# AzheeeQAQ/Game-of-life-distributed

Hardware: AMD Instinct MI355X
Metric: cell-updates/sec (GCUPS) at 1/2/4/8 MI355X; % of HBM roofline (higher is better)
Workload: dtype u32 bit-sliced (1 bit/cell)

## Files before the change

game-of-life-distributed_amd/csrc/gol_kernels.hip:

```cpp
#include "gol_kernels.h"
#include "gol_bits.h"
#include "gol_layout.h"

#include <algorithm>
#include <climits>
#include <type_traits>
#include <utility>

namespace golk {
#ifndef GOL_LOOP_PAD
#define GOL_LOOP_PAD 0
#endif
#ifndef GOL_FILL_PHASES
#define GOL_FILL_PHASES 4
#endif

template <typename F, int... I>
__device__ __forceinline__ void static_for_impl(F &&f, std::integer_sequence<int, I...>) {
    (f(std::integral_constant<int, I>()), ...);
}
template <int N, typename F>
__device__ __forceinline__ void static_for(F &&f) {
    static_for_impl(f, std::make_integer_sequence<int, N>());
}
// ... 447 lines not shown
        if ((threadIdx.x & 63) == 0) atomicAdd(a.alive, (unsigned long long)tot);
    }
}

template <int D, int WPL, bool CNT>
__global__ __launch_bounds__(512) void gol_tb_pair_kernel(StepArgs a) {
    const int lane = threadIdx.x & 63;
    const int w = __builtin_amdgcn_readfirstlane(threadIdx.x >> 6);
    const int tiles_x = (a.Ww + tile_words(WPL) - 1) / tile_words(WPL);
    const int S = a.rows_per_wave;
    const int q = blockIdx.x * 4 + (w & 3);
    const int region = q / tiles_x;
    const int tile = q - region * tiles_x;
    const int r0 = region * 2 * S;
    const int len = r0 < a.rows_out ? min(2 * S, a.rows_out - r0) : 0;
    __shared__ int s_claim[4];
    __shared__ unsigned long long s_cnt;
    if (w < 4 && lane == 0) s_claim[w] = len;
    if (CNT && threadIdx.x == 0) s_cnt = 0;
    __syncthreads();
    if (len == 0) return;
    const uint32_t cnt = stream_band<D, true, WPL, pair_store<WPL>(), true, pair_g2<WPL>()>(a, r0, len, tile * tile_words(WPL), blockIdx.x * 8 + w,
                                                   w < 4 ? 1 : -1, &s_claim[w & 3]);
    if constexpr (!CNT) {
        if (a.alive) {
            const uint32_t tot = wave_sum_u32(cnt);
            if (lane == 0 && tot) atomicAdd(a.alive, (unsigned long long)tot);
        }
    } else if (a.alive) {
        const uint32_t tot = wave_sum_u32(cnt);
        int active = 0;
        for (int i = 0; i < 4; ++i) {
            const int qi = blockIdx.x * 4 + i;
            active += (qi / tiles_x) * 2 * S < a.rows_out ? 2 : 0;
        }
        if (lane == 0) {
            const unsigned long long mine = (1ull << 40) | tot;
            const unsigned long long now = atomicAdd(&s_cnt, mine) + mine;
            const unsigned long long sum = now & ((1ull << 40) - 1);
            if ((int)(now >> 40) == active && sum) atomicAdd(a.alive, sum);
        }
    }
}

__device__ __forceinline__ void wg_count(unsigned long long *alive, unsigned long long *s_cnt, uint32_t cnt, int active) {
    const uint32_t tot = wave_sum_u32(cnt);
    if ((threadIdx.x & 63) == 0) {
        const unsigned long long mine = (1ull << 40) | tot;
        const unsigned long long now = atomicAdd(s_cnt, mine) + mine;
        const unsigned long long sum = now & ((1ull << 40) - 1);
        if ((int)(now >> 40) == active && sum) atomicAdd(alive, sum);
    }
}

template <int WPL>
__device__ __forceinline__ void put_lanes(uint32_t *row, const uint32_t (&v)[WPL]) {
    const int lane = threadIdx.x & 63;
    if constexpr (WPL == 1)
        row[lane] = v[0];
    else if constexpr (WPL == 2)
        reinterpret_cast<uint2 *>(row)[lane] = make_uint2(v[0], v[1]);
    else
        reinterpret_cast<uint4 *>(row)[lane] = make_uint4(v[0], v[1], v[2], v[3]);
}
template <int WPL>
__device__ __forceinline__ Lanes<WPL> get_lanes(const uint32_t *row) {
    const int lane = threadIdx.x & 63;
    Lanes<WPL> v;
    if constexpr (WPL == 1) {
        v.w[0] = row[lane];
    } else if constexpr (WPL == 2) {
        const uint2 q = reinterpret_cast<const uint2 *>(row)[lane];
        v.w[0] = q.x;
        v.w[1] = q.y;
    } else {
        const uint4 q = reinterpret_cast<const uint4 *>(row)[lane];
        v.w[0] = q.x;
        v.w[1] = q.y;
        v.w[2] = q.z;
        v.w[3] = q.w;
    }
    return v;
}
template <int WPL>
__device__ __forceinline__ Lanes<WPL> load_row(const uint32_t *p) {
    Lanes<WPL> v;
    if constexpr (WPL == 1) {
        v.w[0] = *p;
    } else if constexpr (WPL == 2) {
        const uint2 q = *reinterpret_cast<const uint2 *>(p);
        v.w[0] = q.x;
        v.w[1] = q.y;
    } else {
        const uint4 q = *reinterpret_cast<const uint4 *>(p);
        v.w[0] = q.x;
        v.w[1] = q.y;
        v.w[2] = q.z;
        v.w[3] = q.w;
    }
    return v;
}
template <int D, int A, int WPL, typename Hook>
__device__ __forceinline__ void push_group_exp(Lanes<WPL> &x0, Lanes<WPL> &x1, Lanes<WPL> &x2,
                                               uint32_t (&h0)[3][D][WPL], uint32_t (&h1)[3][D][WPL],
                                               uint32_t (&cc)[3][D][WPL], int ii0, Hook &&hook) {
    parity_fix<1>();
#pragma unroll
    for (int s = 0; s < A + 2; ++s) {
        if constexpr (WPL <= 2) parity_fix<1>();
        if (s < A) {
            hook(s, ii0, x0);
            stage<D, 0, WPL>(s, x0, h0, h1, cc);
        }
        if (s >= 1 && s - 1 < A) {
            hook(s - 1, ii0 + 1, x1);
            stage<D, 1, WPL>(s - 1, x1, h0, h1, cc);
        }
        if (s >= 2 && s - 2 < A) {
            hook(s - 2, ii0 + 2, x2);
            stage<D, 2, WPL>(s - 2, x2, h0, h1, cc);
        }
    }
}
#ifndef GOL_SKEW_WAIT_TRACE
#define GOL_SKEW_WAIT_TRACE 0
#endif
#ifndef GOL_SKEW_STORE_CPOL
#define GOL_SKEW_STORE_CPOL 16
#endif
template <int D>
struct SkewPlan {
    static constexpr int STEP = D > 20 ? 6 : 3;
    static constexpr int NPH = (D - 1) / STEP;
    static constexpr int P(int j) { return (j + 1) * STEP; }
    static constexpr int NROWS(int j) { return 2 * ((j + 1 < NPH ? P(j + 1) : D) - P(j)); }
    static constexpr int BASE(int j) {
        int b = 0;
        for (int i = 0; i < j; ++i) b += NROWS(i);
        return b;
    }
    static constexpr int NEXP = BASE(NPH);
    static_assert(NPH >= 1 && STEP % 3 == 0, "skew depth >= 4");
};


template <int D, int WPL>
struct PairSt {
    uint32_t a0[D][WPL], a1[D][WPL];
    uint32_t b0[D][WPL], b1[D][WPL];
    uint32_t p0[D][WPL], p1[D][WPL], p2[D][WPL];
    uint32_t c[D][WPL];
};

template <int D, int PH, int WPL>
__device__ __forceinline__ void stage_pr(int t, Lanes<WPL> &x, PairSt<D, WPL> &st) {
    uint32_t west[WPL], east[WPL];
    if constexpr (WPL == 1) {
        const uint32_t l = from_left_lane(x.w[0]);
        const uint32_t r = from_right_lane(x.w[0]);
        west[0] = __builtin_amdgcn_alignbit(x.w[0], l, 31);
        east[0] = __builtin_amdgcn_alignbit(r, x.w[0], 1);
    } else if constexpr (WPL == 4) {
        const uint32_t l3 = from_left_lane(x.w[3]);
        const uint32_t r0 = from_right_lane(x.w[0]);
        west[0] = __builtin_amdgcn_alignbit(x.w[3], l3, 31);
        west[1] = x.w[0];
        west[2] = x.w[1];
        west[3] = x.w[2];
        east[0] = x.w[1];
        east[1] = x.w[2];
        east[2] = x.w[3];
        east[3] = __builtin_amdgcn_alignbit(r0, x.w[0], 1);
    } else {
        const uint32_t l1 = from_left_lane(x.w[1]);
        const uint32_t r0 = from_right_lane(x.w[0]);
        west[0] = __builtin_amdgcn_alignbit(x.w[1], l1, 31);
        east[0] = x.w[1];
        west[1] = x.w[0];
        east[1] = __builtin_amdgcn_alignbit(r0, x.w[0], 1);
    }
    uint32_t nx[WPL];
#pragma unroll
    for (int k = 0; k < WPL; ++k) {
        const uint32_t n0 = bop<kXor3>(west[k], x.w[k], east[k]);
        const uint32_t n1 = bop<kMaj>(west[k], x.w[k], east[k]);
        if constexpr (PH == 1) {
            uint32_t p0, p1, p2;
            pair_sum(st.b0[t][k], st.b1[t][k], n0, n1, p0, p1, p2);
            nx[k] = pair_rule(st.a0[t][k], st.a1[t][k], p0, p1, p2, st.c[t][k]);
            st.p0[t][k] = p0;
            st.p1[t][k] = p1;
            st.p2[t][k] = p2;
            st.a0[t][k] = n0;
            st.a1[t][k] = n1;
        } else {
            nx[k] = pair_rule(n0, n1, st.p0[t][k], st.p1[t][k], st.p2[t][k], st.c[t][k]);
            st.b0[t][k] = n0;
            st.b1[t][k] = n1;
        }
    }
#pragma unroll
    for (int k = 0; k < WPL; ++k) {
        st.c[t][k] = x.w[k];
        x.w[k] = nx[k];
    }
}

template <int D, int KQ, int WPL>
__device__ __forceinline__ void push_group_pr(Lanes<WPL> &x0, Lanes<WPL> &x1, Lanes<WPL> &x2,
                                              PairSt<D, WPL> &st) {
    parity_fix<1>();
    static_for<D + 2>([&](auto s_tag) {
        constexpr int s = decltype(s_tag)::value;
        parity_fix<2>();
        if constexpr (s < D) stage_pr<D, (KQ + 0 + s) & 1, WPL>(s, x0, st);
        if constexpr (s >= 1 && s - 1 < D) stage_pr<D, (KQ + 1 + s - 1) & 1, WPL>(s - 1, x1, st);
        if constexpr (s >= 2) stage_pr<D, (KQ + 2 + s - 2) & 1, WPL>(s - 2, x2, st);
    });
}

template <int D, int KQ, int LO, int WPL>
__device__ __forceinline__ void push_group_pr_hi(Lanes<WPL> &x0, Lanes<WPL> &x1, Lanes<WPL> &x2,
                                                 PairSt<D, WPL> &st) {
    parity_fix<1>();
    static_for<D + 2>([&](auto s_tag) {
        constexpr int s = decltype(s_tag)::value;
        if constexpr (s >= LO) {
            parity_fix<2>();
            if constexpr (s < D) stage_pr<D, (KQ + 0 + s) & 1, WPL>(s, x0, st);
            if constexpr (s - 1 >= LO && s - 1 < D) stage_pr<D, (KQ + 1 + s - 1) & 1, WPL>(s - 1, x1, st);
            if constexpr (s - 2 >= LO) stage_pr<D, (KQ + 2 + s - 2) & 1, WPL>(s - 2, x2, st);
        }
    });
}

template <int D, int KQ, int WPL>
__device__ __forceinline__ void pr_enter(const uint32_t (&h0)[3][D][WPL], const uint32_t (&h1)[3][D][WPL],
                                         const uint32_t (&cc)[3][D][WPL], PairSt<D, WPL> &st) {
#pragma unroll
    for (int t = 0; t < D; ++t)
#pragma unroll
        for (int k = 0; k < WPL; ++k) {
            st.c[t][k] = cc[2][t][k];
            if (((KQ + t) & 1) == 1) {
                st.a0[t][k] = h0[1][t][k];
                st.a1[t][k] = h1[1][t][k];
                st.b0[t][k] = h0[2][t][k];
                st.b1[t][k] = h1[2][t][k];
            } else {
                pair_sum(h0[1][t][k], h1[1][t][k], h0[2][t][k], h1[2][t][k], st.p0[t][k], st.p1[t][k], st.p2[t][k]);
                st.a0[t][k] = h0[2][t][k];
                st.a1[t][k] = h1[2][t][k];
            }
        }
}
template <int D, int KQ, int WPL>
__device__ __forceinline__ void pr_leave(const PairSt<D, WPL> &st, uint32_t (&h0)[3][D][WPL],
                                         uint32_t (&h1)[3][D][WPL], uint32_t (&cc)[3][D][WPL]) {
#pragma unroll
    for (int t = 0; t < D; ++t)
#pragma unroll
        for (int k = 0; k < WPL; ++k) {
            cc[2][t][k] = st.c[t][k];
            if (((KQ + t) & 1) == 1) {
                h0[1][t][k] = st.a0[t][k];
                h1[1][t][k] = st.a1[t][k];
                h0[2][t][k] = st.b0[t][k];
                h1[2][t][k] = st.b1[t][k];
            } else {
                h0[2][t][k] = st.a0[t][k];
                h1[2][t][k] = st.a1[t][k];
                pair_unsum(st.p0[t][k], st.p1[t][k], st.a0[t][k], st.a1[t][k], h0[1][t][k], h1[1][t][k]);
            }
        }
}

template <int D, int LO, int WPL>
__device__ __forceinline__ void push_group_hi(Lanes<WPL> &x0, Lanes<WPL> &x1, Lanes<WPL> &x2,
                                              uint32_t (&h0)[3][D][WPL], uint32_t (&h1)[3][D][WPL],
                                              uint32_t (&cc)[3][D][WPL]) {
    parity_fix<1>();
#pragma unroll
    for (int s = LO; s < D + 2; ++s) {
        parity_fix<2>();
        if (s < D) stage<D, 0, WPL>(s, x0, h0, h1, cc);
        if (s - 1 >= LO && s - 1 < D) stage<D, 1, WPL>(s - 1, x1, h0, h1, cc);
        if (s - 2 >= LO) stage<D, 2, WPL>(s - 2, x2, h0, h1, cc);
    }
}

template <int D, int WPL, bool HALF = false, bool PR = false>
__device__ __forceinline__ uint32_t stream_skew(const StepArgs &a, int ab, int eb, int tile, bool self,
                                                uint32_t *exp_mine, const uint32_t *exp_next, int *flag_mine,
                                                int *flag_next, unsigned *error, unsigned long long *phase_tr,
                                                int dr = 0) {
    using SP = SkewPlan<D>;
    constexpr int ROW = 64 * WPL;
    constexpr int TV = HALF ? kHalfTileValid : kTileValid;
    const int lane = threadIdx.x & 63;
    const int hl = HALF ? (lane & 31) : lane;
    const int rofs = (HALF && lane >= 32) ? dr : 0;
    const int Ww = a.Ww;
    const int S = eb - ab;
    const int t0 = tile * TV * WPL;
    int col = (t0 + WPL * (hl - 1)) % Ww;
    if (col < 0) col += Ww;
    const bool keep = hl >= 1 && hl <= TV && (t0 + WPL * (hl - 1)) < Ww;
    int r = ab + rofs + a.in.off;
    const int wrap = a.in.wrap > 0 ? a.in.wrap : INT_MAX;
    if (a.in.wrap > 0) {
        r %= a.in.wrap;
        if (r < 0) r += a.in.wrap;
    }
    const uint32_t *__restrict__ src = a.src + col;
    auto load_next = [&]() -> Lanes<WPL> {
        const Lanes<WPL> v = load_row<WPL>(src + (size_t)(a.in.base + min(r, a.in.rmax)) * Ww);
        r = (r + 1 == wrap) ? 0 : r + 1;
        return v;
    };
    const __amdgpu_buffer_rsrc_t brs = __builtin_amdgcn_make_buffer_rsrc(
        a.dst + (size_t)(a.dst_base + ab + D) * Ww, (short)0, (S + (HALF ? dr : 0)) * Ww * 4, 0x00020000);
    const int clo = a.count_lo - (ab + D + rofs), chi = a.count_hi - (ab + D + rofs);
    const int colw = col + rofs * Ww;
    uint32_t cnt = 0;
    auto emit = [&](const Lanes<WPL> &y, int oi) {
        const bool ok = keep && (unsigned)oi < (unsigned)S;
        const int off = ok ? (oi * Ww + colw) * 4 : INT_MAX;
        if constexpr (WPL == 1)
            __builtin_amdgcn_raw_buffer_store_b32(y.w[0], brs, off, 0, GOL_SKEW_STORE_CPOL);
        else if constexpr (WPL == 2)
            __builtin_amdgcn_raw_buffer_store_b64((__attribute__((ext_vector_type(2))) unsigned){y.w[0], y.w[1]}, brs,
                                                  off, 0, GOL_SKEW_STORE_CPOL);
        else
            __builtin_amdgcn_raw_buffer_store_b128(
                (__attribute__((ext_vector_type(4))) unsigned){y.w[0], y.w[1], y.w[2], y.w[3]}, brs, off, 0,
                GOL_SKEW_STORE_CPOL);
        uint32_t pc = 0;
#pragma unroll
        for (int k = 0; k < WPL; ++k) pc += __builtin_popcount(y.w[k]);
        cnt += (ok && oi >= clo && oi < chi) ? pc : 0u;
    };
    auto hook = [&](int s, int k, const Lanes<WPL> &x) {
        if (s % SP::STEP != 0 || s == 0 || s / SP::STEP > SP::NPH) return;
        const int j = s / SP::STEP - 1;
        const int m = k - 2 * SP::P(j);
        const int row = (unsigned)m < (unsigned)SP::NROWS(j) ? SP::BASE(j) + m : SP::NEXP;
        put_lanes<WPL>(exp_mine + row * ROW, x.w);
    };

    uint32_t h0[3][D][WPL], h1[3][D][WPL], cc[3][D][WPL];
#pragma unroll
    for (int s = 0; s < 3; ++s)
#pragma unroll
        for (int t = 0; t < D; ++t)
#pragma unroll
            for (int k = 0; k < WPL; ++k) h0[s][t][k] = h1[s][t][k] = cc[s][t][k] = 0u;

    Lanes<WPL> x0 = vmov(load_next()), x1 = vmov(load_next()), x2 = vmov(load_next());
    int k = 0;
    [[maybe_unused]] unsigned long long wt0 = 0, wmain = 0, nmain = 0, wfill = 0, nfill = 0;
    auto fill = [&](auto a_tag) {
        constexpr int A = decltype(a_tag)::value;
        for (; A == D ? k <= 2 * D - 1 : (k + 2) / 2 <= A - 1; k += 3) {
            const Lanes<WPL> n0 = load_next(), n1 = load_next(), n2 = load_next();
            __builtin_amdgcn_sched_barrier(0);
            Lanes<WPL> y0 = x0, y1 = x1, y2 = x2;
            push_group_exp<D, A, WPL>(y0, y1, y2, h0, h1, cc, k, hook);
            if constexpr (A == D) {
                emit(y0, k - 2 * D);
                emit(y1, k + 1 - 2 * D);
                emit(y2, k + 2 - 2 * D);
            }
            __builtin_amdgcn_sched_barrier(0);
            if constexpr (GOL_SKEW_WAIT_TRACE) wt0 = __builtin_amdgcn_s_memrealtime();
            x0 = vmov(n0);
            x1 = vmov(n1);
            x2 = vmov(n2);
            if constexpr (GOL_SKEW_WAIT_TRACE) {
                asm volatile("s_waitcnt vmcnt(0)" ::: "memory");
                wfill += __builtin_amdgcn_s_memrealtime() - wt0;
                ++nfill;
            }
        }
    };
    static_for<SP::NPH>([&](auto j) { fill(std::integral_constant<int, SP::P(decltype(j)::value)>()); });
    fill(std::integral_constant<int, D>());
    if (phase_tr && lane == 0) phase_tr[0] = (unsigned long long)__builtin_amdgcn_s_memrealtime();
    asm volatile("s_waitcnt lgkmcnt(0)" ::: "memory");
    if (lane == 0) __hip_atomic_store(flag_mine, 1, __ATOMIC_RELAXED, __HIP_MEMORY_SCOPE_WORKGROUP);

    Lanes<WPL> q0, q1, q2;
#pragma unroll
    for (int i = 0; i < WPL; ++i) q0.w[i] = q1.w[i] = q2.w[i] = 0u;
    int qoi = -8;
    [[maybe_unused]] PairSt<D, WPL> st;
    const int kmain = S + (self ? 2 * D : 2 * SP::P(0));
    for (int i = 0; i < GOL_LOOP_PAD; ++i) asm volatile("s_nop 0");
    if constexpr (PR) {
        constexpr int KSTART = 3 * ((2 * D + 2) / 3);
        static_assert(KSTART % 6 == 0, "the pair main loop starts at an even push");
        {
            pr_enter<D, 0, WPL>(h0, h1, cc, st);
            for (; k < kmain; k += 6) {
                {
                    const Lanes<WPL> n0 = load_next(), n1 = load_next(), n2 = load_next();
                    emit(q0, qoi);
                    emit(q1, qoi + 1);
                    emit(q2, qoi + 2);
                    __builtin_amdgcn_sched_barrier(0);
                    Lanes<WPL> y0 = x0, y1 = x1, y2 = x2;
                    push_group_pr<D, 0, WPL>(y0, y1, y2, st);
                    q0 = y0;
                    q1 = y1;
                    q2 = y2;
                    qoi = k - 2 * D;
                    __builtin_amdgcn_sched_barrier(0);
                    x0 = vmov(n0);
                    x1 = vmov(n1);
                    x2 = vmov(n2);
                }
                {
                    const Lanes<WPL> n0 = load_next(), n1 = load_next(), n2 = load_next();
                    emit(q0, qoi);
                    emit(q1, qoi + 1);
                    emit(q2, qoi + 2);
                    __builtin_amdgcn_sched_barrier(0);
                    Lanes<WPL> y0 = x0, y1 = x1, y2 = x2;
                    push_group_pr<D, 1, WPL>(y0, y1, y2, st);
                    q0 = y0;
                    q1 = y1;
                    q2 = y2;
                    qoi = k + 3 - 2 * D;
                    __builtin_amdgcn_sched_barrier(0);
                    x0 = vmov(n0);
                    x1 = vmov(n1);
                    x2 = vmov(n2);
                }
            }
            if constexpr (D % 3 != 0) pr_leave<D, 0, WPL>(st, h0, h1, cc);
        }
    }
    for (; !PR && k < kmain; k += 3) {
        const Lanes<WPL> n0 = load_next(), n1 = load_next(), n2 = load_next();
        emit(q0, qoi);
        emit(q1, qoi + 1);
        emit(q2, qoi + 2);
        __builtin_amdgcn_sched_barrier(0);
        Lanes<WPL> y0 = x0, y1 = x1, y2 = x2;
        push_group<D, D, WPL>(y0, y1, y2, h0, h1, cc);
        q0 = y0;
        q1 = y1;
        q2 = y2;
        qoi = k - 2 * D;
        __builtin_amdgcn_sched_barrier(0);
        if constexpr (GOL_SKEW_WAIT_TRACE) wt0 = __builtin_amdgcn_s_memrealtime();
        x0 = vmov(n0);
        x1 = vmov(n1);
        x2 = vmov(n2);
        if constexpr (GOL_SKEW_WAIT_TRACE) {
            asm volatile("s_waitcnt vmcnt(3)" ::: "memory");
            wmain += __builtin_amdgcn_s_memrealtime() - wt0;
            ++nmain;
        }
    }
    if constexpr (GOL_SKEW_WAIT_TRACE) {
        if (phase_tr && lane == 0) {
            phase_tr[32] = wmain;
            phase_tr[33] = nmain;
            phase_tr[64] = wfill;
            phase_tr[65] = nfill;
        }
    }
    if (phase_tr && lane == 0) phase_tr[1] = (unsigned long long)__builtin_amdgcn_s_memrealtime();
    if (!self) {
        if (__hip_atomic_load(flag_next, __ATOMIC_RELAXED, __HIP_MEMORY_SCOPE_WORKGROUP) == 0) {
            const long long t_start = (long long)__builtin_amdgcn_s_memrealtime();
            while (__hip_atomic_load(flag_next, __ATOMIC_RELAXED, __HIP_MEMORY_SCOPE_WORKGROUP) == 0) {
                if ((long long)__builtin_amdgcn_s_memrealtime() - t_start > 200000000ll) {
                    if (error && lane == 0) __hip_atomic_store(error, 1u, __ATOMIC_RELAXED, __HIP_MEMORY_SCOPE_SYSTEM);
                    break;
                }
                __builtin_amdgcn_s_sleep(1);
            }
        }
        asm volatile("s_waitcnt lgkmcnt(0)" ::: "memory");
        auto imports = [&](int kg, Lanes<WPL> &y0, Lanes<WPL> &y1, Lanes<WPL> &y2) {
            const int d = kg - S;
            int base = SP::BASE(0) - 2 * SP::P(0);
            static_for<SP::NPH>([&](auto j) {
                constexpr int J = decltype(j)::value;
                if (J > 0 && d >= 2 * SP::P(J)) base = SP::BASE(J) - 2 * SP::P(J);
            });
            const int top = SP::NEXP - 1;
            y0 = get_lanes<WPL>(exp_next + min(base + d, top) * ROW);
            y1 = get_lanes<WPL>(exp_next + min(base + d + 1, top) * ROW);
            y2 = get_lanes<WPL>(exp_next + min(base + d + 2, top) * ROW);
        };
        {
            Lanes<WPL> n0, n1, n2;
            imports(k, n0, n1, n2);
            x0 = vmov(n0);
            x1 = vmov(n1);
            x2 = vmov(n2);
        }
        auto drain_pr = [&](auto kq_tag, auto lo_tag) {
            constexpr int KQ = decltype(kq_tag)::value, LO = decltype(lo_tag)::value;
            Lanes<WPL> n0, n1, n2;
            imports(k + 3, n0, n1, n2);
            __builtin_amdgcn_sched_barrier(0);
            Lanes<WPL> y0 = x0, y1 = x1, y2 = x2;
            push_group_pr_hi<D, KQ, LO, WPL>(y0, y1, y2, st);
            parity_fix<1>();
            emit(q0, qoi);
            emit(q1, qoi + 1);
            emit(q2, qoi + 2);
            q0 = y0;
            q1 = y1;
            q2 = y2;
            qoi = k - 2 * D;
            __builtin_amdgcn_sched_barrier(0);
            x0 = vmov(n0);
            x1 = vmov(n1);
            x2 = vmov(n2);
            k += 3;
        };
        auto drain = [&](auto lo_tag, int kend) {
            constexpr int LO = decltype(lo_tag)::value;
            if constexpr (PR && D % 3 == 0) {
                if constexpr (LO == SP::P(SP::NPH - 1) && D - LO <= 6) {
                    static_for<(D - LO) / 3>([&](auto) {
                        drain_pr(std::integral_constant<int, 0>(), lo_tag);
                        drain_pr(std::integral_constant<int, 1>(), lo_tag);
                    });
                    return;
                }
                while (k < kend) {
                    drain_pr(std::integral_constant<int, 0>(), lo_tag);
                    drain_pr(std::integral_constant<int, 1>(), lo_tag);
                }
                return;
            }
            for (; k < kend; k += 3) {
                Lanes<WPL> n0, n1, n2;
                imports(k + 3, n0, n1, n2);
                __builtin_amdgcn_sched_barrier(0);
                Lanes<WPL> y0 = x0, y1 = x1, y2 = x2;
                push_group_hi<D, LO, WPL>(y0, y1, y2, h0, h1, cc);
                __builtin_amdgcn_sched_barrier(0);
                emit(q0, qoi);
                emit(q1, qoi + 1);
                emit(q2, qoi + 2);
                q0 = y0;
                q1 = y1;
                q2 = y2;
                qoi = k - 2 * D;
                __builtin_amdgcn_sched_barrier(0);
                x0 = vmov(n0);
                x1 = vmov(n1);
                x2 = vmov(n2);
            }
        };
        static_for<SP::NPH>([&](auto j) {
            constexpr int J = decltype(j)::value;
            drain(std::integral_constant<int, SP::P(J)>(), S + 2 * (J + 1 < SP::NPH ? SP::P(J + 1) : D));
        });
    }
    emit(q0, qoi);
    emit(q1, qoi + 1);
    emit(q2, qoi + 2);
    return cnt;
}

template <int D, int WPL, bool HALF = false, bool PR = false>
__global__ __launch_bounds__(512) void gol_skew_kernel(SkewArgs p) {
    using SP = SkewPlan<D>;
    constexpr int ROW = 64 * WPL;
    __shared__ uint32_t s_exp[8][(SP::NEXP + 1) * ROW];
    __shared__ int s_flag[8];
    __shared__ unsigned long long s_cnt;
    const int lane = threadIdx.x & 63;
    const int w = __builtin_amdgcn_readfirstlane(threadIdx.x >> 6);
    const int sy = 8 / p.tx;
    const int tcols = (p.tiles_x + p.tx - 1) / p.tx;
    const int stack = blockIdx.x / tcols, tc = blockIdx.x - stack * tcols;
    const int tile = tc * p.tx + w % p.tx, pos = w / p.tx;
    if (lane == 0) s_flag[w] = 0;
    if (threadIdx.x == 0) s_cnt = 0;
    __syncthreads();
    if (tile >= p.tiles_x) return;
    if (p.prio_young && w >= 4) __builtin_amdgcn_s_setprio(1);
    const int L = HALF ? p.base.rows_out / 2 : p.base.rows_out;
    const int A0 = (int)((int64_t)stack * L / p.nst) - D, E0 = (int)((int64_t)(stack + 1) * L / p.nst) - D;
    const int64_t Ls = (int64_t)(E0 - A0) + p.hcap;
    int cum = 0, tot = 0;
    for (int q = 0; q < sy; ++q) {
        tot += p.wgt[q];
        cum += q < pos ? p.wgt[q] : 0;
    }
    const bool bottom = pos == sy - 1;
    constexpr int G = PR ? 6 : 3;
    const int ab = A0 + (int)(Ls * cum / tot) / G * G;
    const int eb = bottom ? E0 : A0 + (int)(Ls * (cum + p.wgt[pos]) / tot) / G * G;
    const long long t_start = p.trace ? (long long)__builtin_amdgcn_s_memrealtime() : 0;
    const uint32_t cnt = stream_skew<D, WPL, HALF, PR>(p.base, ab, eb, tile, bottom, s_exp[w], bottom ? nullptr : s_exp[w + p.tx],
                                             &s_flag[w], bottom ? nullptr : &s_flag[w + p.tx], p.error,
                                             (p.trace && blockIdx.x < 1024) ? p.trace + 8 + 2 * (blockIdx.x * 64 + 16 + w)
                                                                            : nullptr,
                                             L);
    if (p.trace && lane == 0 && blockIdx.x < 1024) {
        p.trace[8 + 2 * (blockIdx.x * 64 + w)] = (unsigned long long)t_start;
        p.trace[8 + 2 * (blockIdx.x * 64 + w) + 1] = (unsigned long long)__builtin_amdgcn_s_memrealtime();
    }
    if (p.base.alive) wg_count(p.base.alive, &s_cnt, cnt, sy * min(p.tx, p.tiles_x - tc * p.tx));
}

__host__ __device__ constexpr int persist_waves(int depth, int wpl) { return depth * wpl <= 16 ? 16 : 8; }

#ifndef GOL_PERSIST_WG_COUNT
#define GOL_PERSIST_WG_COUNT 1
#endif
template <int D, int WPL, int NW>
__global__ __launch_bounds__(NW * 64) void gol_persist_kernel(PersistArgs p) {
    const int lane = threadIdx.x & 63;
    const int w = __builtin_amdgcn_readfirstlane(threadIdx.x >> 6);
    const int b = blockIdx.x;
    const int wx = b % p.cols, wy = b / p.cols;
    const int tile = wx * p.wg_tx + w % p.wg_tx;
    int r0, band, dir = 1;
    const int ry = w / p.wg_tx;
    const bool paired = p.paired != 0;
    if (paired) {
        const int hr = p.wg_sy / 2;
        r0 = wy * p.wg_sy * p.S + 2 * (ry % hr) * p.S;
        band = 2 * p.S;
        dir = ry < hr ? 1 : -1;
    } else if (p.S_old > 0) {
        const int hr = p.wg_sy / 2;
        const int base = wy * p.wg_sy * p.S;
        r0 = base + (ry < hr ? ry * p.S_old : hr * p.S_old + (ry - hr) * p.S_young);
        band = ry < hr ? p.S_old : p.S_young;
        if (ry == p.wg_sy - 1) band = base + p.wg_sy * p.S - r0;
    } else {
        r0 = (wy * p.wg_sy + ry) * p.S;
        band = p.S;
    }
    const int rows_here = (tile < p.tiles_x && r0 < p.base.rows_out) ? min(band, p.base.rows_out - r0) : 0;

    int nb = b;
    if (lane < 9) {
        const int ny = (wy + lane / 3 - 1 + p.wg_y) % p.wg_y;
        const int nx = (wx + lane % 3 - 1 + p.cols) % p.cols;
        nb = ny * p.cols + nx;
    }
    __shared__ int s_abort;
    __shared__ int s_claim[2][NW / 2];
#if GOL_PERSIST_WG_COUNT
    __shared__ unsigned long long s_cnt;
    if (threadIdx.x == 0) s_cnt = 0;
#endif
    if (threadIdx.x == 0) s_abort = 0;
    if (paired && w < NW / 2 && lane == 0) s_claim[0][w] = rows_here;
    __syncthreads();

    uint32_t cnt = 0;
    long long tr_wait = 0, tr_band = 0, tr_max = 0;
    const long long tr_t0 = (long long)__builtin_amdgcn_s_memrealtime();
    for (int j = 0; j < p.J; ++j) {
        const long long tr_w0 = (long long)__builtin_amdgcn_s_memrealtime();
        if (j > 0) {
            if (w == NW - 1) {
                const long long t_start = (long long)__builtin_amdgcn_s_memrealtime();
                for (;;) {
                    const unsigned v = __hip_atomic_load(&p.progress[nb], __ATOMIC_RELAXED, __HIP_MEMORY_SCOPE_AGENT);
                    if (__all(v >= (unsigned)j)) break;
// ... 1635 lines not shown
```

game-of-life-distributed_amd/csrc/golhip.hip:

```cpp
#include <hip/hip_runtime.h>
#include <rccl/rccl.h>

#include <algorithm>
#include <climits>
#include <functional>
#include <atomic>
#include <cstdarg>
#include <cstdio>
#include <cstring>
#include <mutex>
#include <string>
#include <vector>

#include "../../include/golhip.h"
#include "gol_kernels.h"

using golk::kHalo;

namespace {

thread_local std::string g_err;

struct HostBuf {
    uintptr_t base;
// ... 454 lines not shown
    h->ev_pending.clear();
    return GOLHIP_OK;
}

void plan(int strip_rows, int nranks, int rank, int depth, int Ww, golhip_halo_plan_t *p) {
    p->prev_rank = (rank - 1 + nranks) % nranks;
    p->next_rank = (rank + 1) % nranks;
    p->rows = depth;
    p->send_up_row = kHalo;
    p->recv_bottom_row = kHalo + strip_rows;
    p->send_down_row = kHalo + strip_rows - depth;
    p->recv_top_row = kHalo - depth;
    p->bytes = (int64_t)depth * Ww * 4;
}

int exchange_rccl(golhip_t h, int depth, hipStream_t st) {
    if (h->halo_skip) return GOLHIP_OK;
    golhip_halo_plan_t p;
    plan(h->rows, h->nranks, h->rank, depth, h->Ww, &p);
    uint32_t *b = h->buf[h->cur];
    const size_t n = (size_t)depth * h->Ww;
    hipEvent_t e0 = nullptr, e1 = nullptr;
    if (h->flags & GOLHIP_FLAG_TIMING) {
        e0 = take_event(h);
        e1 = take_event(h);
        if (!e0 || !e1) return fail(GOLHIP_EHIP, "hipEventCreate failed");
        HIP_OR_FAIL(hipEventRecord(e0, st));
    }
    if (h->xport) {
        if ((int64_t)n > h->xport_cap) {
            HIP_OR_FAIL(hipHostFree(h->xport_host));
            h->xport_host = nullptr;
            h->xport_cap = 0;
            HIP_OR_FAIL(hipHostMalloc(&h->xport_host, 4 * n * 4, hipHostMallocDefault));
            h->xport_cap = (int64_t)n;
        }
        uint32_t *hb = h->xport_host;
        const size_t bytes = n * 4;
        HIP_OR_FAIL(hipMemcpyAsync(hb, b + (int64_t)p.send_up_row * h->Ww, bytes, hipMemcpyDeviceToHost, st));
        HIP_OR_FAIL(hipMemcpyAsync(hb + n, b + (int64_t)p.send_down_row * h->Ww, bytes, hipMemcpyDeviceToHost, st));
        HIP_OR_FAIL(hipStreamSynchronize(st));
        if (int r = h->xport(h->xport_user, p.prev_rank, p.next_rank, hb, hb + n, hb + 2 * n, hb + 3 * n,
                             (int64_t)bytes))
            return fail(GOLHIP_ERCCL, "test transport returned %d", r);
        HIP_OR_FAIL(hipMemcpyAsync(b + (int64_t)p.recv_top_row * h->Ww, hb + 2 * n, bytes, hipMemcpyHostToDevice, st));
        HIP_OR_FAIL(hipMemcpyAsync(b + (int64_t)p.recv_bottom_row * h->Ww, hb + 3 * n, bytes, hipMemcpyHostToDevice, st));
        HIP_OR_FAIL(hipStreamSynchronize(st));
    } else {
        NCCL_OR_FAIL(ncclGroupStart());
        NCCL_OR_FAIL(ncclSend(b + (int64_t)p.send_up_row * h->Ww, n, ncclUint32, p.prev_rank, h->comm, st));
        NCCL_OR_FAIL(ncclRecv(b + (int64_t)p.recv_bottom_row * h->Ww, n, ncclUint32, p.next_rank, h->comm, st));
        NCCL_OR_FAIL(ncclSend(b + (int64_t)p.send_down_row * h->Ww, n, ncclUint32, p.next_rank, h->comm, st));
        NCCL_OR_FAIL(ncclRecv(b + (int64_t)p.recv_top_row * h->Ww, n, ncclUint32, p.prev_rank, h->comm, st));
        NCCL_OR_FAIL(ncclGroupEnd());
    }
    if (e1) {
        HIP_OR_FAIL(hipEventRecord(e1, st));
        h->ev_pending.push_back({e0, e1, 3});
    }
    h->halo_bytes += 2 * (int64_t)n * 4;
    h->halo_exchanges++;
    return GOLHIP_OK;
}

void shift_rows(golk::StepArgs &a, int lo, int hi) {
    const int rows = a.rows_out;
    a.rows_out = hi - lo;
    a.dst_base = kHalo + lo;
    a.in.off = kHalo + lo;
    a.dummy_rows = std::max(1, std::min(a.dummy_rows, kHalo + std::min(lo, 0)));
    a.count_lo = -lo;
    a.count_hi = -lo + rows;
}

int skew_bpc(golhip_t h, int depth, int wpl, bool half, bool pr) {
    int &c = h->skew_bpc[depth_index(depth)][(wpl == 4 ? 2 : wpl - 1) + (half ? 3 : 0) + (pr ? 6 : 0)];
    if (c == 0) {
        const int b = golk::skew_blocks_per_cu(depth, wpl, half, pr);
        c = b > 0 ? b : -1;
    }
    return c;
}

bool skew_dims(golhip_t h, int depth, int wpl, int L, golk::SkewArgs *sk) {
    const bool pr = depth == 18 || (wpl == 4 && depth == 8 && (h->skew_pairs & 2));
    if (!h->skew || h->W % 32 != 0 || !golk::skew_supported(depth, wpl, false, pr)) return false;
    const int hcap = h->skew_hcap >= 0 ? h->skew_hcap : 3 * depth / 4;
    const int smin = depth + 3;
    const bool half_ok = h->skew_half >= 0 && L % 2 == 0 && golk::skew_supported(depth, wpl, true, pr);
    int best_tx = 0, best_nst = 0, best_half = 0, best_tiles = 0;
    double best = 1e300;
    for (int half = 0; half <= (half_ok ? 1 : 0); ++half) {
        if (!half && half_ok && h->skew_half > 0) continue;
        const int bpc = skew_bpc(h, depth, wpl, half, pr);
        if (bpc < 1) continue;
        const int tiles = half ? (h->Ww + golk::kHalfTileValid * wpl - 1) / (golk::kHalfTileValid * wpl)
                               : golk::tb_tiles(h->Ww, wpl);
        const int Lh = half ? L / 2 : L;
        for (int tx = 1; tx <= 2; ++tx) {
            if (h->skew_tx && tx != h->skew_tx) continue;
            const int sy = 8 / tx, tcols = (tiles + tx - 1) / tx;
            const int nst = std::min(h->cu_count * bpc / tcols,
                                     Lh / (sy * (smin + hcap) - hcap));
            if (nst < 1) continue;
            if (h->skew == 1 && (int64_t)nst * tcols * 4 < (int64_t)h->cu_count * bpc * 3) continue;
            if (((double)Lh / nst + hcap + (half ? Lh : 0)) * h->Ww * 4 >= 2147483648.0) continue;
            const double per_wave = ((double)Lh / nst + hcap) / sy * (half ? 1.02 : 1.0);
            if (per_wave < best * 0.999) {
                best = per_wave;
                best_tx = tx;
                best_nst = nst;
                best_half = half;
                best_tiles = tiles;
            }
        }
    }
    if (!best_tx) return false;
    sk->tiles_x = best_tiles;
    sk->pairs = pr ? 1 : 0;
    sk->tx = best_tx;
    sk->nst = best_nst;
    sk->half = best_half;
    sk->hcap = hcap;
    return true;
}

bool skew_fills(golhip_t h) {
    if (!h->skew || h->W % 32 != 0) return false;
    const int wpl = wpl_per_launch(h);
    int cap = std::min(h->tb_depth, golk::max_depth_for(wpl));
    if (cap == 9 && wpl != 4) cap = 8;
    const int depth = cap == 9 ? 9 : largest_depth(cap);
    golk::SkewArgs sk{};
    return skew_dims(h, depth, wpl, sched_rows(h), &sk);
}

bool skew_plan(golhip_t h, int depth, int wpl, const golk::StepArgs &a, golk::SkewArgs *sk) {
    if (!skew_dims(h, depth, wpl, a.rows_out, sk)) return false;
    if (!h->skew_err) {
        void *p = nullptr, *d = nullptr;
        if (hipHostMalloc(&p, sizeof(unsigned), hipHostMallocMapped) != hipSuccess) return false;
        if (hipHostGetDevicePointer(&d, p, 0) != hipSuccess) {
            (void)hipHostFree(p);
            return false;
        }
        h->skew_err = static_cast<unsigned *>(p);
        h->skew_err_dev = static_cast<unsigned *>(d);
        *h->skew_err = 0;
    }
    const int sy = 8 / sk->tx;
    const int young = h->skew_young > 0 ? h->skew_young
                      : wpl == 4             ? 78
                      : sk->half             ? 60
                      : a.in.wrap > 0        ? 70
                                             : 68;
    for (int q = 0; q < 8; ++q) sk->wgt[q] = (q < sy && q * sk->tx >= 4) ? young : 100;
    sk->prio_young = h->skew_prio;
    sk->error = h->skew_err_dev;
    sk->trace = h->d_trace;
    return true;
}

int launch_rows(golhip_t h, int depth, unsigned long long *alive, bool halo, int lo, int hi) {
    const hipStream_t st = h->stream;
    golk::StepArgs a = step_args(h, alive, halo);
    if (lo != 0 || hi != h->rows) shift_rows(a, lo, hi);
    const int wpl = wpl_for(h);
    if (a.rows_out == h->rows) {
        a.rows_per_wave = rows_per_wave_for(h, depth);
    } else if (h->rows_per_wave > 0) {
        a.rows_per_wave = h->rows_per_wave;
    } else {
        const int slots = h->cu_count * golk::tb_wave_slots_per_cu(depth, wpl, tb_paired(h));
        a.rows_per_wave = golk::auto_rows_per_wave(h->Ww, a.rows_out, depth, std::max(slots, 1), h->fill_skip, wpl,
                                                     tb_paired(h));
    }
    a.rows_per_wave = (int)std::min<int64_t>(a.rows_per_wave, ((1ll << 31) - 1) / (8ll * h->Ww));
    hipEvent_t e0 = nullptr, e1 = nullptr;
    if (h->flags & GOLHIP_FLAG_TIMING) {
        e0 = take_event(h);
        e1 = take_event(h);
        if (!e0 || !e1) return fail(GOLHIP_EHIP, "hipEventCreate failed");
        HIP_OR_FAIL(hipEventRecord(e0, st));
    }
    hipError_t e;
    golk::SkewArgs sk{};
    const bool skew = skew_plan(h, depth, wpl, a, &sk);
    if (skew) {
        sk.base = a;
        e = golk::launch_skew(sk, depth, wpl, st);
    } else if (h->W % 32 == 0) {
        e = golk::launch_step_tb(a, depth, st, h->fill_skip, wpl, tb_paired(h));
    } else {
        e = golk::launch_step_generic(a, st);
    }
    h->last_variant = h->W % 32 != 0 ? 0 : skew ? 3 : 1;
    if (e != hipSuccess) return fail(GOLHIP_EHIP, "step launch: %s", hipGetErrorString(e));
    if (e1) {
        HIP_OR_FAIL(hipEventRecord(e1, st));
        h->ev_pending.push_back({e0, e1, 0});
        if (h->ev_pending.size() >= 4096) {
            int rc = drain_events(h);
            if (rc) return rc;
        }
    }
    h->step_launches++;
    h->skew_launches += skew;
    h->skew_half_launches += skew && sk.half;
    if (skew && sk.pairs) {
        h->pair_launches++;
        h->pair_turns += depth;
    }
    return GOLHIP_OK;
}

void finish_launch(golhip_t h, int depth, bool count) {
    h->cur ^= 1;
    h->turns += depth;
    h->step_turns += depth;
    if (count) h->alive_turn = h->turns;
}

int launch_depth(golhip_t h, int depth, bool count, bool halo) {
    unsigned long long *alive = nullptr;
    if (count) {
        alive = h->d_scalars;
        HIP_OR_FAIL(hipMemsetAsync(alive, 0, sizeof(unsigned long long), h->stream));
    }
    if (int rc = launch_rows(h, depth, alive, halo, 0, h->rows)) return rc;
    finish_launch(h, depth, count);
    return GOLHIP_OK;
}

int halo_launches(int rows, int depth, int64_t run) {
    const int64_t k = std::min<int64_t>({(int64_t)kHalo / depth, run, (int64_t)rows / depth});
    return (int)std::max<int64_t>(1, k);
}

struct HaloRun {
    int d, k;
};
HaloRun halo_next(int cap, int rows, bool resident, int64_t left) {
    DepthRun run = depth_plan(cap, left);
    if (resident) {
        const int d = largest_depth(std::min<int64_t>(cap, left));
        run = {d, left / d};
    }
    return {run.d, halo_launches(rows, run.d, run.n)};
}

int launch_ext(golhip_t h, int depth, bool count, int ext) {
    unsigned long long *alive = nullptr;
    if (count) {
        alive = h->d_scalars;
        HIP_OR_FAIL(hipMemsetAsync(alive, 0, sizeof(unsigned long long), h->stream));
    }
    if (int rc = launch_rows(h, depth, alive, true, -ext, h->rows + ext)) return rc;
    finish_launch(h, depth, count);
    return GOLHIP_OK;
}

int check_persist(golhip_t h) {
    if (!h->persist_pending) return GOLHIP_OK;
    h->persist_pending = false;
    if (*h->h_err) {
        *h->h_err = 0;
        h->persistent = 0;
        return fail(GOLHIP_EHIP, "persistent step kernel timed out waiting for a neighbour workgroup "
                                 "(not all workgroups resident?); board state is undefined, persistent mode disabled");
    }
    return GOLHIP_OK;
}

bool measurement_env() {
    const char *v = getenv("GOLHIP_MEASUREMENT");
    return v && !strcmp(v, "1");
}
bool test_hooks_env() {
    const char *v = getenv("GOLHIP_TEST_HOOKS");
    return v && !strcmp(v, "1");
}
constexpr const char *kTuningKeys[] = {
    "persist_depth", "persist_waves", "dummy_rows", "paired_bands", "persist_half", "persist_wg_tx", "trace",
    "cu_count", "fill_skip", "skew_young", "skew_hcap", "skew_prio", "skew_half", "skew_tx", "lds_depth",
    "lds_waves", "lds_wg_cu", "lds_age", "lds_pre", "lds_stride", "lds_xcd", "flip_overlap", "skew_pairs"};
bool tuning_env() {
    const char *v = getenv("GOLHIP_TUNING");
    return (v && !strcmp(v, "1")) || measurement_env();
}
constexpr const char *kConsentInfo =
    " CONSENT_MEASUREMENT=halo_skip,flip_debug:1-3"
    " CONSENT_TEST_HOOKS=resident_fault,resident_max_turns,flip_debug:4,golhip_test_ring_init"
    " CONSENT_TUNING=persist_depth,persist_waves,dummy_rows,paired_bands,persist_half,persist_wg_tx,trace,cu_count,"
    "fill_skip,skew_young,skew_hcap,skew_prio,skew_half,skew_tx,lds_depth,lds_waves,lds_wg_cu,lds_age,lds_pre,"
    "lds_stride,lds_xcd,flip_overlap,skew_pairs"
    " PRODUCT_OPTIONS=wpl,persistent,lds_band,skew,timing,persist_timeout_us,force_halo";

int take_skew_err(golhip_t h) {
    if (h->skew_err && *h->skew_err) {
        *h->skew_err = 0;
        return fail(GOLHIP_EHIP, "skewed-band step kernel: a band waited past its spin bound for the band below "
                                 "(board state is undefined)");
    }
    return GOLHIP_OK;
}

int sync_stream(golhip_t h) {
// ... 2148 lines not shown
```

Baseline: 138,800.

## Software-pipeline cross-lane row shifts into the previous stage's LUT stream

Restructures the pair-rule stage into a unit that computes the west/east cross-lane shifts (DPP moves plus alignbit) for the next row while the current row's logic ops run, placing them at fixed points inside the instruction window with sched barriers. This is meant to hide DPP/alignbit latency and data hazards behind independent bitwise work. It reorders the stage sequence across the three rows, uses wave_shr/wave_shl DPP variants, adds odd/even-sized vmov padding for instruction alignment, and raises the young-wave weight for wrapped pair runs. The risk is extra register pressure and tighter coupling to hand-tuned instruction placement.

```diff
diff --git a/game-of-life-distributed_amd/csrc/gol_kernels.hip b/game-of-life-distributed_amd/csrc/gol_kernels.hip
--- a/game-of-life-distributed_amd/csrc/gol_kernels.hip
+++ b/game-of-life-distributed_amd/csrc/gol_kernels.hip
@@ -623,53 +623,89 @@
     uint32_t c[D][WPL];
 };
 
+struct Shifted {
+    uint32_t w, e;
+};
+template <int WPL>
+__device__ __forceinline__ Shifted row_shifts(const Lanes<WPL> &x) {
+    const uint32_t l = from_left_lane(x.w[WPL - 1]);
+    const uint32_t r = from_right_lane(x.w[0]);
+    return {__builtin_amdgcn_alignbit(x.w[WPL - 1], l, 31), __builtin_amdgcn_alignbit(r, x.w[0], 1)};
+}
+__device__ __forceinline__ uint32_t from_left_lane_far(uint32_t v) {
+    uint32_t r;
+    asm volatile("v_mov_b32_dpp %0, %1 wave_shr:1 row_mask:0xf bank_mask:0xf bound_ctrl:1" : "=v"(r) : "v"(v));
+    return r;
+}
+__device__ __forceinline__ uint32_t from_right_lane_far(uint32_t v) {
+    uint32_t r;
+    asm volatile("v_mov_b32_dpp %0, %1 wave_shl:1 row_mask:0xf bank_mask:0xf bound_ctrl:1" : "=v"(r) : "v"(v));
+    return r;
+}
+template <int WPL>
+__device__ __forceinline__ Lanes<WPL> vmov_even(const Lanes<WPL> &v) {
+    static_assert(WPL % 2 == 0, "s_waitcnt + one 8-byte move + an odd number of 4-byte ones");
+    Lanes<WPL> r;
+    asm volatile("v_mov_b32_e64 %0, %1" : "=v"(r.w[0]) : "v"(v.w[0]));
+#pragma unroll
+    for (int k = 1; k < WPL; ++k) asm volatile("v_mov_b32 %0, %1" : "=v"(r.w[k]) : "v"(v.w[k]));
+    return r;
+}
+
 template <int D, int PH, int WPL>
-__device__ __forceinline__ void stage_pr(int t, Lanes<WPL> &x, PairSt<D, WPL> &st) {
-    uint32_t west[WPL], east[WPL];
-    if constexpr (WPL == 1) {
-        const uint32_t l = from_left_lane(x.w[0]);
-        const uint32_t r = from_right_lane(x.w[0]);
-        west[0] = __builtin_amdgcn_alignbit(x.w[0], l, 31);
-        east[0] = __builtin_amdgcn_alignbit(r, x.w[0], 1);
-    } else if constexpr (WPL == 4) {
-        const uint32_t l3 = from_left_lane(x.w[3]);
-        const uint32_t r0 = from_right_lane(x.w[0]);
-        west[0] = __builtin_amdgcn_alignbit(x.w[3], l3, 31);
-        west[1] = x.w[0];
-        west[2] = x.w[1];
-        west[3] = x.w[2];
-        east[0] = x.w[1];
-        east[1] = x.w[2];
-        east[2] = x.w[3];
-        east[3] = __builtin_amdgcn_alignbit(r0, x.w[0], 1);
-    } else {
-        const uint32_t l1 = from_left_lane(x.w[1]);
-        const uint32_t r0 = from_right_lane(x.w[0]);
-        west[0] = __builtin_amdgcn_alignbit(x.w[1], l1, 31);
-        east[0] = x.w[1];
-        west[1] = x.w[0];
-        east[1] = __builtin_amdgcn_alignbit(r0, x.w[0], 1);
-    }
-    uint32_t nx[WPL];
-#pragma unroll
-    for (int k = 0; k < WPL; ++k) {
-        const uint32_t n0 = bop<kXor3>(west[k], x.w[k], east[k]);
-        const uint32_t n1 = bop<kMaj>(west[k], x.w[k], east[k]);
-        if constexpr (PH == 1) {
-            uint32_t p0, p1, p2;
-            pair_sum(st.b0[t][k], st.b1[t][k], n0, n1, p0, p1, p2);
-            nx[k] = pair_rule(st.a0[t][k], st.a1[t][k], p0, p1, p2, st.c[t][k]);
-            st.p0[t][k] = p0;
-            st.p1[t][k] = p1;
-            st.p2[t][k] = p2;
-            st.a0[t][k] = n0;
-            st.a1[t][k] = n1;
+__device__ __forceinline__ void unit_pr(int t, Lanes<WPL> &x, const Shifted sh, PairSt<D, WPL> &st,
+                                        const Lanes<WPL> &xn, Shifted &shn) {
+    constexpr int OPS = PH == 1 ? 10 : 6;
+    constexpr int NL = OPS * WPL, NW = (NL + 4) / 4;
+    static_assert(NL % 4 == 0, "whole windows: 4 shifts + a multiple of 4 LUTs");
+    uint32_t l = 0, r = 0;
+    uint32_t n0[WPL], n1[WPL], u0[WPL], u1[WPL], u2[WPL], u3[WPL], s7[WPL], nx[WPL];
+    static_for<NL>([&](auto j_tag) {
+        constexpr int j = decltype(j_tag)::value, k = j / OPS, op = j % OPS;
+        if constexpr (op <= 1) {
+            uint32_t west, east;
+            if constexpr (k == 0) west = sh.w; else west = x.w[k - 1];
+            if constexpr (k == WPL - 1) east = sh.e; else east = x.w[k + 1];
+            if constexpr (op == 0) n0[k] = bop<kXor3>(west, x.w[k], east);
+            if constexpr (op == 1) n1[k] = bop<kMaj>(west, x.w[k], east);
+        } else if constexpr (PH == 1) {
+            if constexpr (op == 2) u0[k] = bop<kXor2>(st.b0[t][k], n0[k], n0[k]);
+            if constexpr (op == 3) u2[k] = bop<kAnd2>(st.b0[t][k], n0[k], n0[k]);
+            if constexpr (op == 4) u1[k] = bop<kXor3>(st.b1[t][k], n1[k], u2[k]);
+            if constexpr (op == 5) u3[k] = bop<kMaj>(st.b1[t][k], n1[k], u2[k]);
+            if constexpr (op == 6) u2[k] = bop<kPrA>(st.a0[t][k], u0[k], st.c[t][k]);
+            if constexpr (op == 7) s7[k] = bop<kPrB>(st.a1[t][k], u1[k], u3[k]);
+            if constexpr (op == 8) u2[k] = bop<kPrC>(st.c[t][k], u2[k], s7[k]);
+            if constexpr (op == 9) {
+                nx[k] = bop<kPrNext>(u3[k], s7[k], u2[k]);
+                st.p0[t][k] = u0[k];
+                st.p1[t][k] = u1[k];
+                st.p2[t][k] = u3[k];
+                st.a0[t][k] = n0[k];
+                st.a1[t][k] = n1[k];
+            }
         } else {
-            nx[k] = pair_rule(n0, n1, st.p0[t][k], st.p1[t][k], st.p2[t][k], st.c[t][k]);
-            st.b0[t][k] = n0;
-            st.b1[t][k] = n1;
-        }
-    }
+            if constexpr (op == 2) u2[k] = bop<kPrA>(n0[k], st.p0[t][k], st.c[t][k]);
+            if constexpr (op == 3) s7[k] = bop<kPrB>(n1[k], st.p1[t][k], st.p2[t][k]);
+            if constexpr (op == 4) u2[k] = bop<kPrC>(st.c[t][k], u2[k], s7[k]);
+            if constexpr (op == 5) {
+                nx[k] = bop<kPrNext>(st.p2[t][k], s7[k], u2[k]);
+                st.b0[t][k] = n0[k];
+                st.b1[t][k] = n1[k];
+            }
+        }
+        static_for<4>([&](auto i_tag) {
+            constexpr int i = decltype(i_tag)::value;
+            if constexpr (j + 1 == 4 * (i * NW / 4) - i + 3) {
+                __builtin_amdgcn_sched_barrier(0);
+                if constexpr (i == 0) l = from_left_lane_far(xn.w[WPL - 1]);
+                if constexpr (i == 1) shn.w = __builtin_amdgcn_alignbit(xn.w[WPL - 1], l, 31);
+                if constexpr (i == 2) r = from_right_lane_far(xn.w[0]);
+                if constexpr (i == 3) shn.e = __builtin_amdgcn_alignbit(r, xn.w[0], 1);
+                __builtin_amdgcn_sched_barrier(0);
+            }
+        });
+    });
 #pragma unroll
     for (int k = 0; k < WPL; ++k) {
         st.c[t][k] = x.w[k];
@@ -677,32 +713,38 @@
     }
 }
 
-template <int D, int KQ, int WPL>
-__device__ __forceinline__ void push_group_pr(Lanes<WPL> &x0, Lanes<WPL> &x1, Lanes<WPL> &x2,
-                                              PairSt<D, WPL> &st) {
-    parity_fix<1>();
-    static_for<D + 2>([&](auto s_tag) {
-        constexpr int s = decltype(s_tag)::value;
-        parity_fix<2>();
-        if constexpr (s < D) stage_pr<D, (KQ + 0 + s) & 1, WPL>(s, x0, st);
-        if constexpr (s >= 1 && s - 1 < D) stage_pr<D, (KQ + 1 + s - 1) & 1, WPL>(s - 1, x1, st);
-        if constexpr (s >= 2) stage_pr<D, (KQ + 2 + s - 2) & 1, WPL>(s - 2, x2, st);
-    });
-}
-
 template <int D, int KQ, int LO, int WPL>
 __device__ __forceinline__ void push_group_pr_hi(Lanes<WPL> &x0, Lanes<WPL> &x1, Lanes<WPL> &x2,
-                                                 PairSt<D, WPL> &st) {
+                                                 PairSt<D, WPL> &st, Shifted &sh, const Lanes<WPL> &n0,
+                                                 Lanes<WPL> &xn) {
     parity_fix<1>();
-    static_for<D + 2>([&](auto s_tag) {
-        constexpr int s = decltype(s_tag)::value;
-        if constexpr (s >= LO) {
-            parity_fix<2>();
-            if constexpr (s < D) stage_pr<D, (KQ + 0 + s) & 1, WPL>(s, x0, st);
-            if constexpr (s - 1 >= LO && s - 1 < D) stage_pr<D, (KQ + 1 + s - 1) & 1, WPL>(s - 1, x1, st);
-            if constexpr (s - 2 >= LO) stage_pr<D, (KQ + 2 + s - 2) & 1, WPL>(s - 2, x2, st);
+    Shifted nx;
+    unit_pr<D, (KQ + 0 + LO) & 1, WPL>(LO, x0, sh, st, x1, nx);
+    sh = nx;
+    static_for<D - LO>([&](auto t_tag) {
+        constexpr int t = LO + decltype(t_tag)::value;
+        parity_fix<2>();
+        if constexpr (t + 1 < D) {
+            unit_pr<D, (KQ + 1 + t) & 1, WPL>(t, x1, sh, st, x0, nx);
+            sh = nx;
+            unit_pr<D, (KQ + 0 + t + 1) & 1, WPL>(t + 1, x0, sh, st, x2, nx);
+            sh = nx;
+            unit_pr<D, (KQ + 2 + t) & 1, WPL>(t, x2, sh, st, x1, nx);
+            sh = nx;
+        } else {
+            unit_pr<D, (KQ + 1 + t) & 1, WPL>(t, x1, sh, st, x2, nx);
+            sh = nx;
+            xn = vmov_even(n0);
+            __builtin_amdgcn_sched_barrier(0);
+            unit_pr<D, (KQ + 2 + t) & 1, WPL>(t, x2, sh, st, xn, nx);
+            sh = nx;
         }
     });
+}
+template <int D, int KQ, int WPL>
+__device__ __forceinline__ void push_group_pr(Lanes<WPL> &x0, Lanes<WPL> &x1, Lanes<WPL> &x2, PairSt<D, WPL> &st,
+                                              Shifted &sh, const Lanes<WPL> &n0, Lanes<WPL> &xn) {
+    push_group_pr_hi<D, KQ, 0, WPL>(x0, x1, x2, st, sh, n0, xn);
 }
 
 template <int D, int KQ, int WPL>
@@ -865,6 +907,7 @@
     for (int i = 0; i < WPL; ++i) q0.w[i] = q1.w[i] = q2.w[i] = 0u;
     int qoi = -8;
     [[maybe_unused]] PairSt<D, WPL> st;
+    [[maybe_unused]] Shifted sh = {0u, 0u};
     const int kmain = S + (self ? 2 * D : 2 * SP::P(0));
     for (int i = 0; i < GOL_LOOP_PAD; ++i) asm volatile("s_nop 0");
     if constexpr (PR) {
@@ -872,6 +915,7 @@
         static_assert(KSTART % 6 == 0, "the pair main loop starts at an even push");
         {
             pr_enter<D, 0, WPL>(h0, h1, cc, st);
+            sh = row_shifts<WPL>(x0);
             for (; k < kmain; k += 6) {
                 {
                     const Lanes<WPL> n0 = load_next(), n1 = load_next(), n2 = load_next();
@@ -880,14 +924,15 @@
                     emit(q2, qoi + 2);
                     __builtin_amdgcn_sched_barrier(0);
                     Lanes<WPL> y0 = x0, y1 = x1, y2 = x2;
-                    push_group_pr<D, 0, WPL>(y0, y1, y2, st);
+                    Lanes<WPL> xn;
+                    push_group_pr<D, 0, WPL>(y0, y1, y2, st, sh, n0, xn);
                     q0 = y0;
                     q1 = y1;
                     q2 = y2;
                     qoi = k - 2 * D;
                     __builtin_amdgcn_sched_barrier(0);
-                    x0 = vmov(n0);
-                    x1 = vmov(n1);
+                    x0 = xn;
+                    if constexpr (HALF) x1 = vmov(n1); else x1 = vmov_even(n1);
                     x2 = vmov(n2);
                 }
                 {
@@ -897,13 +942,14 @@
                     emit(q2, qoi + 2);
                     __builtin_amdgcn_sched_barrier(0);
                     Lanes<WPL> y0 = x0, y1 = x1, y2 = x2;
-                    push_group_pr<D, 1, WPL>(y0, y1, y2, st);
+                    Lanes<WPL> xn;
+                    push_group_pr<D, 1, WPL>(y0, y1, y2, st, sh, n0, xn);
                     q0 = y0;
                     q1 = y1;
                     q2 = y2;
                     qoi = k + 3 - 2 * D;
                     __builtin_amdgcn_sched_barrier(0);
-                    x0 = vmov(n0);
+                    x0 = xn;
                     x1 = vmov(n1);
                     x2 = vmov(n2);
                 }
@@ -973,6 +1019,7 @@
             x0 = vmov(n0);
             x1 = vmov(n1);
             x2 = vmov(n2);
+            if constexpr (PR && D % 3 == 0) sh = row_shifts<WPL>(x0);
         }
         auto drain_pr = [&](auto kq_tag, auto lo_tag) {
             constexpr int KQ = decltype(kq_tag)::value, LO = decltype(lo_tag)::value;
@@ -980,7 +1027,8 @@
             imports(k + 3, n0, n1, n2);
             __builtin_amdgcn_sched_barrier(0);
             Lanes<WPL> y0 = x0, y1 = x1, y2 = x2;
-            push_group_pr_hi<D, KQ, LO, WPL>(y0, y1, y2, st);
+            Lanes<WPL> xn;
+            push_group_pr_hi<D, KQ, LO, WPL>(y0, y1, y2, st, sh, n0, xn);
             parity_fix<1>();
             emit(q0, qoi);
             emit(q1, qoi + 1);
@@ -990,7 +1038,7 @@
             q2 = y2;
             qoi = k - 2 * D;
             __builtin_amdgcn_sched_barrier(0);
-            x0 = vmov(n0);
+            x0 = xn;
             x1 = vmov(n1);
             x2 = vmov(n2);
             k += 3;
diff --git a/game-of-life-distributed_amd/csrc/golhip.hip b/game-of-life-distributed_amd/csrc/golhip.hip
--- a/game-of-life-distributed_amd/csrc/golhip.hip
+++ b/game-of-life-distributed_amd/csrc/golhip.hip
@@ -630,7 +630,7 @@
     const int young = h->skew_young > 0 ? h->skew_young
                       : wpl == 4             ? 78
                       : sk->half             ? 60
-                      : a.in.wrap > 0        ? 70
+                      : a.in.wrap > 0        ? (sk->pairs ? 80 : 70)
                                              : 68;
     for (int q = 0; q < 8; ++q) sk->wgt[q] = (q < sy && q * sk->tx >= 4) ? young : 100;
     sk->prio_young = h->skew_prio;
```

New measurement: 145,700, median of 6. 4.9% higher.
